# fhausmann/deepgrp

Hardware: AMD Instinct MI355X
Metric: Mbp/sec predicted (whole node) at window=200 stride=50, 5-class (higher is better)
Workload: dtype f16

## Files before the change

deepgrp_amd/csrc/gru_split2.hip:

```cpp
#include "gru_shared.h"
#include <mutex>
#include <type_traits>

typedef unsigned u32x4 __attribute__((ext_vector_type(4)));

namespace {

constexpr int NW = 4, UP = 128, KS = 4, HPAD = 16, HS = UP + HPAD;
constexpr int XT_PITCH = 4 * 128 * 4 + 32;

struct split2_weights {
    u32x4 hi[3][KS][2], lo[3][KS][2];
    u32x4 Bd_hi, Bd_lo;
};

#define LOAD2(a, pa, b, pb)                                                                                             \
    asm volatile("global_load_dwordx4 %0, %2, off\n\tglobal_load_dwordx4 %1, %3, off\n\ts_waitcnt vmcnt(0)"            \
                 : "=&a"(a), "=&a"(b) : "v"(pa), "v"(pb) : "memory")

#define MFMA_R(acc, Wf, b) asm volatile("v_mfma_f32_16x16x32_f16 %0, %1, %2, %0" : "+v"(acc) : "a"(Wf), "v"(b))
#define MFMA_D(acc, a, Wf) asm volatile("v_mfma_f32_16x16x32_f16 %0, %1, %2, %0" : "+v"(acc) : "v"(a), "a"(Wf))
#define MFMA_DZ(acc, a, Wf) asm volatile("v_mfma_f32_16x16x32_f16 %0, %1, %2, 0" : "=&v"(acc) : "v"(a), "a"(Wf))

struct tile_state {
    gru_params p;
    wg_ctx ctx;
    unsigned hcur, hnxt, lcur, lnxt;
    unsigned myseq;
    float h[16];
    f32x4 ar[4], ag[4], az[4], ax[4];
    f32x4 dpl;
    unsigned tabf, tabr;
    half8 f0h[2], f0l[2];
    int p_off;
    int64_t p_row0;
    bool pr_on;
};

template <int MODE, bool ONERCP>
__global__ void __launch_bounds__(256) __attribute__((amdgpu_waves_per_eu(1, 1))) gru_split2_kernel(const gru_params pin, int half_bytes)
{
    extern __shared__ __attribute__((aligned(16))) unsigned char smem[];
    const int tid = threadIdx.x;
    const int lane = tid & 63;
    const int wave = __builtin_amdgcn_readfirstlane(tid >> 6);
    const int T = pin.T, C = pin.C;

    split2_weights W;
    {
        const uint4 *p16 = pin.pack16 + (size_t)wave * 48 * 64 + lane;
#pragma unroll
        for (int g = 0; g < 3; ++g)
#pragma unroll
            for (int ks = 0; ks < KS; ++ks) {
                LOAD2(W.hi[g][ks][0], p16 + (size_t)(g * 8 + ks * 2) * 64, W.hi[g][ks][1], p16 + (size_t)(g * 8 + ks * 2 + 1) * 64);
                LOAD2(W.lo[g][ks][0], p16 + (size_t)(24 + g * 8 + ks * 2) * 64, W.lo[g][ks][1], p16 + (size_t)(24 + g * 8 + ks * 2 + 1) * 64);
            }
        const uint4 *mypack = pin.pack + (size_t)wave * pin.nfrag * 64 + lane;
        LOAD2(W.Bd_hi, mypack + (size_t)(3 * (2 * KS + 1) + 1) * 64, W.Bd_lo, mypack + (size_t)(3 * (2 * KS + 1) + 2) * 64);
    }
    for (int i = tid; i < 5 * 512; i += 256)
        *reinterpret_cast<float *>(smem + pin.xtab_off + (i / 512) * XT_PITCH + (i % 512) * 4) = pin.xtab[i];

    const int wi = lane & 15, q4 = lane >> 4;
    const int cls = lane & 15;
    const float fbias = cls < C ? pin.ffb[cls] : 0.0f;
    const int pwi = 4 * (lane >> 4) + wave;
    const unsigned frag_lane = (unsigned)(wi * HS + 8 * q4) * 2;
    const unsigned dense_lane = (unsigned)(wi * HS + 32 * wave + 8 * q4) * 2;
    const unsigned pub_lane = (unsigned)(wi * HS + 32 * wave + 4 * q4) * 2;
    const unsigned tab_lane = (unsigned)pin.xtab_off + (unsigned)(32 * wave + 4 * q4) * 4;

    tile_state S0, S1;
    auto setup = [&](tile_state &Z, int x) {
        unsigned char *base = smem + (size_t)x * half_bytes;
        _Float16 *lbuf = reinterpret_cast<_Float16 *>(base + pin.lo_tile_off);
        for (int i = tid; i < 32 * HS; i += 256) lbuf[i] = (_Float16)0.0f;
        Z.p = pin;
        const int64_t bid = wg_record_at<MODE>(pin, Z.p, 2 * (int64_t)blockIdx.x + x);
        Z.ctx = wg_setup<NW, MODE, HPAD>(Z.p, base, bid);
        Z.hcur = (unsigned)x * half_bytes;
        Z.hnxt = Z.hcur + 32 * HS * 2;
        Z.lcur = (unsigned)x * half_bytes + pin.lo_tile_off;
        Z.lnxt = Z.lcur + 32 * HS * 2;
        Z.myseq = (unsigned)(Z.ctx.seqs - smem) + wi * pin.Tp;
#pragma unroll
        for (int i = 0; i < 16; ++i) Z.h[i] = ONERCP ? -1.0f : 0.0f;
        Z.p_off = Z.ctx.rowoff[pwi];
        Z.p_row0 = Z.ctx.row0s[pwi];
        Z.pr_on = cls < C && pwi < Z.ctx.nvalid;
    };
    setup(S0, 0);
    setup(S1, 1);

    auto lds16 = [&](unsigned off) -> half8 { return *reinterpret_cast<const half8 *>(smem + off); };
    auto ldsf4 = [&](unsigned off) -> f32x4 { return *reinterpret_cast<const f32x4 *>(smem + off); };
    auto tab_rows = [&](tile_state &Z, uint32_t bf, uint32_t br) {
        bf = bf < 4 ? bf : 4;
        br = br < 4 ? 3 - br : 4;
        Z.tabf = tab_lane + bf * XT_PITCH;
        Z.tabr = tab_lane + br * XT_PITCH;
    };
    auto acc_init = [&](tile_state &Z, int g, int sub) {
        const f32x4 v = ldsf4(((sub & 1) ? Z.tabr : Z.tabf) + g * 512 + (sub >> 1) * 64);
        if (g == 0) Z.ar[sub] = v; else if (g == 1) Z.ag[sub] = v; else Z.az[sub] = v;
    };

    struct frag_ring { half8 h[2][2], l[2][2]; };
    struct dense_ops { half8 a0, a1, l0, l1; };
    struct fin_state { float d[NW], lg, m, e, s; };
    auto phase = [&](auto do_x, auto do_y, auto do_f, tile_state &X, tile_state &Y, int tx, int ty) __attribute__((always_inline)) {
        constexpr bool DO_X = decltype(do_x)::value, DO_Y = decltype(do_y)::value, DO_F = decltype(do_f)::value;
        frag_ring F;
        dense_ops D;
        fin_state fs;
        split_gate_tmp gt[16];
        float pbh[4][4];
        uint2 pbhv[4], pblv[4];
        uint32_t xp_bf = 4, xp_br = 4;
        const int td = ty - 1;
        const int tf = tx - 2;
        if constexpr (DO_X) { F.h[0][0] = X.f0h[0]; F.h[0][1] = X.f0h[1]; F.l[0][0] = X.f0l[0]; F.l[0][1] = X.f0l[1]; }
#define GAP __builtin_amdgcn_sched_barrier(0);
#define M_K(ks, n)                                                                                               \
    if constexpr (DO_X) {                                                                                        \
        constexpr int ps_ = (n) / 12, g_ = ((n) % 12) / 4, uh_ = ((n) % 4) / 2, rh_ = (n) % 2, sub_ = 2 * uh_ + rh_; \
        const half8 &b_ = ps_ == 1 ? F.l[(ks) & 1][rh_] : F.h[(ks) & 1][rh_];                                    \
        const u32x4 &w_ = ps_ == 2 ? W.lo[g_][ks][uh_] : W.hi[g_][ks][uh_];                                      \
        if constexpr (g_ == 0) MFMA_R(X.ar[sub_], w_, b_);                                                       \
        else if constexpr (g_ == 1) MFMA_R(X.ag[sub_], w_, b_);                                                  \
        else MFMA_R(X.az[sub_], w_, b_);                                                                         \
    }
#define M_D(i)                                                                                                   \
    if constexpr (DO_X) {                                                                                        \
        if constexpr ((i) == 0) MFMA_DZ(X.dpl, D.a0, W.Bd_hi);                                                   \
        else if constexpr ((i) == 1) MFMA_D(X.dpl, D.a1, W.Bd_hi);                                               \
        else if constexpr ((i) == 2) MFMA_D(X.dpl, D.a0, W.Bd_lo);                                               \
        else if constexpr ((i) == 3) MFMA_D(X.dpl, D.a1, W.Bd_lo);                                               \
        else if constexpr ((i) == 4) MFMA_D(X.dpl, D.l0, W.Bd_hi);                                               \
        else MFMA_D(X.dpl, D.l1, W.Bd_hi);                                                                       \
    }
#define PF(ks)                                                                                                   \
    if constexpr (DO_X) {                                                                                        \
        F.h[(ks) & 1][0] = lds16(X.hcur + frag_lane + 64 * (ks)); F.h[(ks) & 1][1] = lds16(X.hcur + frag_lane + 16 * HS * 2 + 64 * (ks)); \
        F.l[(ks) & 1][0] = lds16(X.lcur + frag_lane + 64 * (ks)); F.l[(ks) & 1][1] = lds16(X.lcur + frag_lane + 16 * HS * 2 + 64 * (ks)); \
    }
#define RDD                                                                                                      \
    if constexpr (DO_X) {                                                                                        \
        D.a0 = lds16(X.hcur + dense_lane); D.a1 = lds16(X.hcur + dense_lane + 16 * HS * 2);                      \
        D.l0 = lds16(X.lcur + dense_lane); D.l1 = lds16(X.lcur + dense_lane + 16 * HS * 2);                      \
        if (MODE == 2 && tx > 0 && (lane & 15) < X.ctx.nvalid)                                                   \
            split_avg_store(X.p, X.ctx.wg_w, tx - 1, UP, wave, D.a0, D.a1, D.l0, D.l1);                          \
    }
#define AXL(sub) \
    if constexpr (DO_Y) Y.ax[sub] = ldsf4((((sub) & 1) ? Y.tabr : Y.tabf) + 3 * 512 + ((sub) >> 1) * 64);
#define DS(i)                                                                                                    \
    if constexpr (DO_Y) Y.ctx.dpart[((size_t)(td & 1) * 4 * NW + wave) * 64 + lane + (i) * NW * 64] = Y.dpl[i];
#define G(e, op) \
    if constexpr (DO_Y) split_gate_op<ONERCP, op>(gt[e], Y.ar[(e) / 4][(e) % 4], Y.ag[(e) / 4][(e) % 4], Y.az[(e) / 4][(e) % 4], Y.ax[(e) / 4][(e) % 4], Y.h[e]);
#define PB(g, op)                                                                                                \
    if constexpr (DO_Y) {                                                                                        \
        if constexpr ((op) == 0) {                                                                               \
            pbh[g][0] = split_state_h<ONERCP>(Y.h[4 * (g)]); pbh[g][1] = split_state_h<ONERCP>(Y.h[4 * (g) + 1]); \
            pbh[g][2] = split_state_h<ONERCP>(Y.h[4 * (g) + 2]); pbh[g][3] = split_state_h<ONERCP>(Y.h[4 * (g) + 3]); \
        } else if constexpr ((op) == 1) {                                                                        \
            pbhv[g] = split_pack4(pbh[g]);                                                                       \
        } else if constexpr ((op) == 2) {                                                                        \
            split_residual4(pbh[g], pbhv[g]);                                                                    \
        } else if constexpr ((op) == 3) {                                                                        \
            pblv[g] = split_pack4(pbh[g]);                                                                       \
        } else {                                                                                                 \
            *reinterpret_cast<uint2 *>(smem + Y.hnxt + pub_lane + ((g) & 1) * 16 * HS * 2 + ((g) >> 1) * 32) = pbhv[g]; \
            *reinterpret_cast<uint2 *>(smem + Y.lnxt + pub_lane + ((g) & 1) * 16 * HS * 2 + ((g) >> 1) * 32) = pblv[g]; \
        }                                                                                                        \
    }
#define BAR                                                                                                      \
    if constexpr (DO_Y) {                                                                                        \
        asm volatile("s_waitcnt lgkmcnt(0)\n\ts_barrier" ::: "memory");                                          \
        unsigned sw_ = Y.hcur; Y.hcur = Y.hnxt; Y.hnxt = sw_;                                                    \
        sw_ = Y.lcur; Y.lcur = Y.lnxt; Y.lnxt = sw_;                                                             \
    }
#define RD0                                                                                                      \
    if constexpr (DO_Y) {                                                                                        \
        Y.f0h[0] = lds16(Y.hcur + frag_lane); Y.f0h[1] = lds16(Y.hcur + frag_lane + 16 * HS * 2);                \
        Y.f0l[0] = lds16(Y.lcur + frag_lane); Y.f0l[1] = lds16(Y.lcur + frag_lane + 16 * HS * 2);                \
    }
#define XP(op)                                                                                                   \
    if constexpr (DO_Y) {                                                                                        \
        if constexpr ((op) == 0) { xp_bf = smem[Y.myseq + ty + 1]; xp_br = smem[Y.myseq + T - 2 - ty]; }                       \
        else tab_rows(Y, xp_bf, xp_br);                                                                          \
    }
#define CI(g, sub) \
    if constexpr (DO_Y) acc_init(Y, g, sub);
#define FN(op)                                                                                                   \
    if constexpr (DO_F) {                                                                                        \
        if constexpr ((op) == 0) {                                                                               \
            const float *dp_ = X.ctx.dpart + ((size_t)(tf & 1) * 4 + wave) * NW * 64 + lane;                     \
            fs.d[0] = dp_[0]; fs.d[1] = dp_[64]; fs.d[2] = dp_[128]; fs.d[3] = dp_[192];                         \
        } else if constexpr ((op) == 1) {                                                                        \
            const float sum_ = ((fs.d[0] + fs.d[1]) + fs.d[2]) + fs.d[3];                                        \
            fs.lg = cls < C ? sum_ + fbias : -INFINITY;                                                          \
        } else if constexpr ((op) == 2) { if (MODE != 2) fs.m = row_max_ror<8>(fs.lg); }                         \
        else if constexpr ((op) == 3) { if (MODE != 2) fs.m = row_max_ror<4>(fs.m); }                            \
        else if constexpr ((op) == 4) { if (MODE != 2) fs.m = row_max_ror<2>(fs.m); }                            \
        else if constexpr ((op) == 5) { if (MODE != 2) fs.m = row_max_ror<1>(fs.m); }                            \
        else if constexpr ((op) == 6) { if (MODE != 2) fs.e = __builtin_amdgcn_exp2f(1.4426950408889634f * (fs.lg - fs.m)); } \
        else if constexpr ((op) == 7) { if (MODE != 2) fs.s = fs.e + row_ror<8>(fs.e); }                         \
        else if constexpr ((op) == 8) { if (MODE != 2) fs.s += row_ror<4>(fs.s); }                               \
        else if constexpr ((op) == 9) { if (MODE != 2) fs.s += row_ror<2>(fs.s); }                               \
        else if constexpr ((op) == 10) { if (MODE != 2) fs.s += row_ror<1>(fs.s); }                              \
        else if constexpr ((op) == 11) { if (MODE != 2) fs.e *= __builtin_amdgcn_rcpf(fs.s); }                   \
        else { if (X.pr_on && tf >= 0) emit_value<MODE>(X.p, X.ctx, X.p_off, X.p_row0, tf, cls, MODE == 2 ? fs.lg : fs.e); } \
    }
#include "gru_split2_phase.inc"
#undef GAP
#undef M_K
#undef M_D
#undef PF
#undef RDD
#undef AXL
#undef DS
#undef G
#undef PB
#undef BAR
#undef RD0
#undef XP
#undef CI
#undef FN
    };
    const std::true_type yes;
    const std::false_type no;

    auto first_step = [&](tile_state &Z) {
        tab_rows(Z, smem[Z.myseq], smem[Z.myseq + T - 1]);
#pragma unroll
        for (int g = 0; g < 3; ++g)
#pragma unroll
            for (int sub = 0; sub < 4; ++sub) acc_init(Z, g, sub);
        Z.f0h[0] = lds16(Z.hcur + frag_lane); Z.f0h[1] = lds16(Z.hcur + frag_lane + 16 * HS * 2);
        Z.f0l[0] = lds16(Z.lcur + frag_lane); Z.f0l[1] = lds16(Z.lcur + frag_lane + 16 * HS * 2);
    };
    first_step(S0);
    first_step(S1);
    phase(yes, no, no, S0, S1, 0, 0);
#define EDGE_PAD do { asm volatile("s_nop 15\n\ts_nop 7"); __builtin_amdgcn_sched_barrier(0); } while (0)
    EDGE_PAD;
    for (int t = 0; t + 1 < T; ++t) {
        phase(yes, yes, yes, S1, S0, t, t);
        phase(yes, yes, yes, S0, S1, t + 1, t);
        EDGE_PAD;
    }
    phase(yes, yes, yes, S1, S0, T - 1, T - 1);
    phase(no, yes, yes, S0, S1, T, T - 1);

    auto drain = [&](tile_state &Z, bool prev_open) {
        const half8 a0 = lds16(Z.hcur + dense_lane), a1 = lds16(Z.hcur + dense_lane + 16 * HS * 2);
        const half8 l0 = lds16(Z.lcur + dense_lane), l1 = lds16(Z.lcur + dense_lane + 16 * HS * 2);
        if (MODE == 2 && (lane & 15) < Z.ctx.nvalid) split_avg_store(Z.p, Z.ctx.wg_w, T - 1, UP, wave, a0, a1, l0, l1);
        f32x4 d;
        MFMA_DZ(d, a0, W.Bd_hi); MFMA_D(d, a1, W.Bd_hi); MFMA_D(d, a0, W.Bd_lo); MFMA_D(d, a1, W.Bd_lo); MFMA_D(d, l0, W.Bd_hi); MFMA_D(d, l1, W.Bd_hi);
        asm volatile("s_nop 15\n\ts_nop 7" : "+v"(d));
        float *dw = Z.ctx.dpart + ((size_t)((T - 1) & 1) * 4 * NW + wave) * 64 + lane;
#pragma unroll
        for (int reg = 0; reg < 4; ++reg) dw[reg * NW * 64] = d[reg];
        __syncthreads();
        if (prev_open && T > 1) finish_register<NW, MODE>(Z.p, Z.ctx, T - 2, wave, fbias, Z.p_off, Z.p_row0);
        finish_register<NW, MODE>(Z.p, Z.ctx, T - 1, wave, fbias, Z.p_off, Z.p_row0);
        if (MODE == 0 && pin.ospan > 0) flush_image<NW>(Z.p, Z.ctx);
    };
    drain(S0, false);
    drain(S1, true);
}

template <int MODE, bool ONERCP>
int launch_split2(const gru_params &p, int64_t groups, int half_bytes, hipStream_t stream)
{
    static std::once_flag configured;
    static hipError_t cfg_err = hipSuccess;
    std::call_once(configured, [] { cfg_err = hipFuncSetAttribute((const void *)gru_split2_kernel<MODE, ONERCP>, hipFuncAttributeMaxDynamicSharedMemorySize, 160 * 1024); });
    DGRP_HIP(cfg_err);
    hipLaunchKernelGGL((gru_split2_kernel<MODE, ONERCP>), dim3((unsigned)((groups + 1) / 2)), dim3(256), (size_t)2 * half_bytes + 5 * XT_PITCH, stream, p, half_bytes);
    DGRP_LAUNCH_CHECK();
    return DGRP_OK;
}

}

int dgrp_split2_launch(const gru_params &p, int64_t groups, int half_bytes, bool onercp, hipStream_t stream)
{
    if (onercp)
        return p.mode == 0 ? launch_split2<0, true>(p, groups, half_bytes, stream)
             : p.mode == 1 ? launch_split2<1, true>(p, groups, half_bytes, stream) : launch_split2<2, true>(p, groups, half_bytes, stream);
    return p.mode == 0 ? launch_split2<0, false>(p, groups, half_bytes, stream)
         : p.mode == 1 ? launch_split2<1, false>(p, groups, half_bytes, stream) : launch_split2<2, false>(p, groups, half_bytes, stream);
}
```

Baseline: 550.2.

## Overlap GRU kernel prologue loads with LDS setup and batch weight loads

Restructures the kernel prologue. The global loads of the x-table and the sequence bytes are issued early into registers and committed to LDS after the weight loads. The weight fragments now load in batches of sixteen dwordx4 per asm block instead of pairs with a wait after each pair, and the wg_setup call is inlined into separate place, fill, row and commit stages with 16-byte zero fills. This aims to hide prologue memory latency before the recurrent loop, at the cost of more register pressure during the prologue and more complex sequence-staging code. It also adds optional timestamp instrumentation, compiled only under a define.

```diff
diff --git a/deepgrp_amd/csrc/gru_split2.hip b/deepgrp_amd/csrc/gru_split2.hip
--- a/deepgrp_amd/csrc/gru_split2.hip
+++ b/deepgrp_amd/csrc/gru_split2.hip
@@ -37,6 +37,25 @@
     bool pr_on;
 };
 
+#ifdef DGRP_SPLIT2_STAMPS
+#define SPLIT2_STAMP(k)                                                                                          \
+    do {                                                                                                         \
+        __builtin_amdgcn_sched_barrier(0);                                                                       \
+        if (MODE == 0 && pin.avg) {                                                                              \
+            unsigned long long c_, r_;                                                                           \
+            asm volatile("s_memtime %0\n\ts_memrealtime %1\n\ts_waitcnt lgkmcnt(0)" : "=s"(c_), "=s"(r_) :: "memory"); \
+            if (threadIdx.x == 0) {                                                                              \
+                unsigned long long *b_ = reinterpret_cast<unsigned long long *>(pin.avg) + (size_t)blockIdx.x * 16; \
+                b_[2 * (k)] = c_; b_[2 * (k) + 1] = r_;                                                          \
+                if ((k) == 0) { b_[10] = __builtin_amdgcn_s_getreg(4 | (31 << 11)); b_[11] = __builtin_amdgcn_s_getreg(20 | (31 << 11)); } \
+            }                                                                                                    \
+        }                                                                                                        \
+        __builtin_amdgcn_sched_barrier(0);                                                                       \
+    } while (0)
+#else
+#define SPLIT2_STAMP(k) do { } while (0)
+#endif
+
 template <int MODE, bool ONERCP>
 __global__ void __launch_bounds__(256) __attribute__((amdgpu_waves_per_eu(1, 1))) gru_split2_kernel(const gru_params pin, int half_bytes)
 {
@@ -46,25 +65,9 @@
     const int wave = __builtin_amdgcn_readfirstlane(tid >> 6);
     const int T = pin.T, C = pin.C;
 
-    split2_weights W;
-    {
-        const uint4 *p16 = pin.pack16 + (size_t)wave * 48 * 64 + lane;
-#pragma unroll
-        for (int g = 0; g < 3; ++g)
-#pragma unroll
-            for (int ks = 0; ks < KS; ++ks) {
-                LOAD2(W.hi[g][ks][0], p16 + (size_t)(g * 8 + ks * 2) * 64, W.hi[g][ks][1], p16 + (size_t)(g * 8 + ks * 2 + 1) * 64);
-                LOAD2(W.lo[g][ks][0], p16 + (size_t)(24 + g * 8 + ks * 2) * 64, W.lo[g][ks][1], p16 + (size_t)(24 + g * 8 + ks * 2 + 1) * 64);
-            }
-        const uint4 *mypack = pin.pack + (size_t)wave * pin.nfrag * 64 + lane;
-        LOAD2(W.Bd_hi, mypack + (size_t)(3 * (2 * KS + 1) + 1) * 64, W.Bd_lo, mypack + (size_t)(3 * (2 * KS + 1) + 2) * 64);
-    }
-    for (int i = tid; i < 5 * 512; i += 256)
-        *reinterpret_cast<float *>(smem + pin.xtab_off + (i / 512) * XT_PITCH + (i % 512) * 4) = pin.xtab[i];
-
+    SPLIT2_STAMP(0);
     const int wi = lane & 15, q4 = lane >> 4;
     const int cls = lane & 15;
-    const float fbias = cls < C ? pin.ffb[cls] : 0.0f;
     const int pwi = 4 * (lane >> 4) + wave;
     const unsigned frag_lane = (unsigned)(wi * HS + 8 * q4) * 2;
     const unsigned dense_lane = (unsigned)(wi * HS + 32 * wave + 8 * q4) * 2;
@@ -72,26 +75,173 @@
     const unsigned tab_lane = (unsigned)pin.xtab_off + (unsigned)(32 * wave + 4 * q4) * 4;
 
     tile_state S0, S1;
-    auto setup = [&](tile_state &Z, int x) {
+    auto place = [&](tile_state &Z, int x) {
         unsigned char *base = smem + (size_t)x * half_bytes;
-        _Float16 *lbuf = reinterpret_cast<_Float16 *>(base + pin.lo_tile_off);
-        for (int i = tid; i < 32 * HS; i += 256) lbuf[i] = (_Float16)0.0f;
         Z.p = pin;
         const int64_t bid = wg_record_at<MODE>(pin, Z.p, 2 * (int64_t)blockIdx.x + x);
-        Z.ctx = wg_setup<NW, MODE, HPAD>(Z.p, base, bid);
+        wg_ctx &c = Z.ctx;
+        c.hbuf = reinterpret_cast<_Float16 *>(base);
+        c.dpart = reinterpret_cast<float *>(base + gru_lds_hbuf(UP, HPAD));
+        c.seqs = base + gru_lds_hbuf(UP, HPAD) + gru_lds_dpart(NW);
+        c.row0s = reinterpret_cast<int64_t *>(c.seqs + gru_lds_seq(pin.Tp));
+        c.rowoff = reinterpret_cast<int *>(c.row0s + DGRP_WG_WINDOWS);
+        c.obuf = reinterpret_cast<unsigned *>(c.rowoff + DGRP_WG_WINDOWS);
+        c.wg_w = Z.p.w0 + bid * DGRP_WG_WINDOWS;
+        c.nvalid = (int)min((int64_t)DGRP_WG_WINDOWS, Z.p.w0 + Z.p.nw - c.wg_w);
+        c.lo = 0;
+        if (MODE == 0) {
+            const int64_t a = dgrp_place_row(Z.p.place, c.wg_w, Z.p.s), b = dgrp_place_row(Z.p.place, c.wg_w + c.nvalid - 1, Z.p.s);
+            c.lo = a < b ? a : b;
+        }
         Z.hcur = (unsigned)x * half_bytes;
         Z.hnxt = Z.hcur + 32 * HS * 2;
         Z.lcur = (unsigned)x * half_bytes + pin.lo_tile_off;
         Z.lnxt = Z.lcur + 32 * HS * 2;
+    };
+    place(S0, 0);
+    place(S1, 1);
+
+    constexpr int SEQ_R = 2;
+    const bool span_form = pin.s <= (int64_t)T && 15 * pin.s + 2 * (int64_t)T + 16 <= (int64_t)gru_lds_seq(pin.Tp);
+    struct seq_regs { uint32_t dw[SEQ_R]; uint8_t by; };
+    auto seq_geom = [&](const tile_state &Z, const uint8_t *&g4, int &al, int &len) {
+        const int nv = Z.ctx.nvalid > 0 ? Z.ctx.nvalid : 0;
+        const uint8_t *g = Z.p.idx + Z.ctx.wg_w * Z.p.s;
+        al = (int)(reinterpret_cast<uintptr_t>(g) & 3);
+        g4 = g - al;
+        len = nv > 0 ? (nv - 1) * (int)Z.p.s + T : 0;
+    };
+    auto seq_issue = [&](const tile_state &Z, seq_regs &Q) {
+        const uint8_t *g4; int al, len;
+        seq_geom(Z, g4, al, len);
+#pragma unroll
+        for (int r = 0; r < SEQ_R; ++r) {
+            const int k = tid + 256 * r;
+            Q.dw[r] = 0;
+            if (4 * k >= al && 4 * k + 4 <= al + len) Q.dw[r] = reinterpret_cast<const uint32_t *>(g4)[k];
+        }
+        const int kl = (al + len - 1) >> 2, k = tid < 4 ? 0 : kl, j = 4 * k + (tid & 3) - al;
+        Q.by = 0;
+        if (tid < 8 && (tid < 4 || kl > 0) && j >= 0 && j < len && !(4 * k >= al && 4 * k + 4 <= al + len)) Q.by = g4[al + j];
+    };
+    auto seq_commit = [&](tile_state &Z, const seq_regs &Q) {
+        const uint8_t *g4; int al, len;
+        seq_geom(Z, g4, al, len);
+        unsigned char *dst = Z.ctx.seqs + 4;
+#pragma unroll
+        for (int r = 0; r < SEQ_R; ++r) {
+            const int k = tid + 256 * r;
+            if (4 * k >= al && 4 * k + 4 <= al + len) reinterpret_cast<uint32_t *>(dst)[k] = Q.dw[r];
+        }
+        const int kl = (al + len - 1) >> 2, k = tid < 4 ? 0 : kl, j = 4 * k + (tid & 3) - al;
+        if (tid < 8 && (tid < 4 || kl > 0) && j >= 0 && j < len && !(4 * k >= al && 4 * k + 4 <= al + len)) dst[al + j] = Q.by;
+        for (int k0 = 256 * SEQ_R; 4 * k0 < al + len; k0 += 4 * 256) {
+            uint32_t v[4];
+#pragma unroll
+            for (int r = 0; r < 4; ++r) {
+                const int kk = k0 + tid + 256 * r;
+                v[r] = 4 * kk + 4 <= al + len ? reinterpret_cast<const uint32_t *>(g4)[kk] : 0u;
+            }
+#pragma unroll
+            for (int r = 0; r < 4; ++r) {
+                const int kk = k0 + tid + 256 * r;
+                if (4 * kk + 4 <= al + len) reinterpret_cast<uint32_t *>(dst)[kk] = v[r];
+            }
+        }
+        const int fours = (al + len + 3) & ~3;
+        for (int i = tid; 4 * i < T; i += 256) reinterpret_cast<uint32_t *>(dst + fours)[i] = 0x04040404u;
+        Z.myseq = (unsigned)(dst - smem) + (wi < Z.ctx.nvalid ? al + wi * (int)Z.p.s : fours);
+    };
+    auto seq_rows = [&](tile_state &Z) {
+        const int w = tid >> 4;
+        const bool on = w < Z.ctx.nvalid;
+        const uint8_t *g = Z.p.idx + (Z.ctx.wg_w + w) * Z.p.s;
+        for (int t0 = tid & 15; t0 < T; t0 += 8 * 16) {
+            uint8_t v[8];
+#pragma unroll
+            for (int r = 0; r < 8; ++r) v[r] = on && t0 + 16 * r < T ? g[t0 + 16 * r] : (uint8_t)4;
+#pragma unroll
+            for (int r = 0; r < 8; ++r)
+                if (t0 + 16 * r < T) Z.ctx.seqs[w * pin.Tp + t0 + 16 * r] = v[r];
+        }
         Z.myseq = (unsigned)(Z.ctx.seqs - smem) + wi * pin.Tp;
+    };
+
+    const f32x4 *xsrc = reinterpret_cast<const f32x4 *>(pin.xtab) + tid;
+    const f32x4 xt0 = xsrc[0], xt1 = xsrc[256];
+    f32x4 xt2 = { 0.0f, 0.0f, 0.0f, 0.0f };
+    if (tid < 5 * 128 - 512) xt2 = xsrc[512];
+    seq_regs Q0, Q1;
+    if (span_form) { seq_issue(S0, Q0); seq_issue(S1, Q1); }
+    const float fbias = cls < C ? pin.ffb[cls] : 0.0f;
+    auto zero16 = [&](unsigned char *at, int bytes) {
+        for (int i = tid; i < bytes / 16; i += 256) reinterpret_cast<uint4 *>(at)[i] = uint4{ 0u, 0u, 0u, 0u };
+        if (tid < (bytes & 15) / 4) reinterpret_cast<unsigned *>(at + (bytes & ~15))[tid] = 0u;
+    };
+    auto fills = [&](tile_state &Z) {
+        zero16(smem + Z.hcur, 32 * HS * 2);
+        zero16(smem + Z.lcur, 32 * HS * 2);
+        if (MODE == 0) zero16(reinterpret_cast<unsigned char *>(Z.ctx.obuf), pin.ospan * C * 4);
+    };
+    fills(S0);
+    fills(S1);
+
+    split2_weights W;
+    {
+        const uint4 *p16 = pin.pack16 + (size_t)wave * 48 * 64 + lane;
+#define WF(f) ((f) < 24 ? W.hi[((f) % 24) / 8][((f) % 8) / 2][(f) % 2] : W.lo[((f) % 24) / 8][((f) % 8) / 2][(f) % 2])
+#define GLD(o, a, off) "global_load_dwordx4 %" #o ", %" #a ", off offset:" #off "\n\t"
+#define GLD8(o0, o1, o2, o3, o4, o5, o6, o7, a) \
+    GLD(o0, a, -4096) GLD(o1, a, -3072) GLD(o2, a, -2048) GLD(o3, a, -1024) GLD(o4, a, 0) GLD(o5, a, 1024) GLD(o6, a, 2048) GLD(o7, a, 3072)
+#define LOAD16(f)                                                                                                          \
+    asm volatile(GLD8(0, 1, 2, 3, 4, 5, 6, 7, 16) GLD8(8, 9, 10, 11, 12, 13, 14, 15, 17) "s_waitcnt vmcnt(0)"            \
+                 : "=&a"(WF((f) + 0)), "=&a"(WF((f) + 1)), "=&a"(WF((f) + 2)), "=&a"(WF((f) + 3)), "=&a"(WF((f) + 4)), "=&a"(WF((f) + 5)),     \
+                   "=&a"(WF((f) + 6)), "=&a"(WF((f) + 7)), "=&a"(WF((f) + 8)), "=&a"(WF((f) + 9)), "=&a"(WF((f) + 10)), "=&a"(WF((f) + 11)),  \
+                   "=&a"(WF((f) + 12)), "=&a"(WF((f) + 13)), "=&a"(WF((f) + 14)), "=&a"(WF((f) + 15))                     \
+                 : "v"(p16 + (size_t)((f) + 4) * 64), "v"(p16 + (size_t)((f) + 12) * 64) : "memory")
+        LOAD16(0);
+        LOAD16(16);
+        LOAD16(32);
+#undef LOAD16
+#undef GLD8
+#undef GLD
+#undef WF
+        const uint4 *mypack = pin.pack + (size_t)wave * pin.nfrag * 64 + lane;
+        LOAD2(W.Bd_hi, mypack + (size_t)(3 * (2 * KS + 1) + 1) * 64, W.Bd_lo, mypack + (size_t)(3 * (2 * KS + 1) + 2) * 64);
+    }
+    SPLIT2_STAMP(1);
+
+    auto xrow = [&](int i) { return reinterpret_cast<f32x4 *>(smem + pin.xtab_off + (i >> 7) * XT_PITCH + (i & 127) * 16); };
+    *xrow(tid) = xt0;
+    *xrow(tid + 256) = xt1;
+    if (tid < 5 * 128 - 512) *xrow(tid + 512) = xt2;
+    if (span_form) { seq_commit(S0, Q0); seq_commit(S1, Q1); }
+    else { seq_rows(S0); seq_rows(S1); }
+    auto rows = [&](tile_state &Z) {
+        const wg_ctx &c = Z.ctx;
+        if (tid < DGRP_WG_WINDOWS) {
+            int64_t r0 = -1;
+            int off = -1;
+            if (tid < c.nvalid) {
+                r0 = MODE == 0 ? dgrp_place_row(Z.p.place, c.wg_w + tid, Z.p.s) : (c.wg_w + tid - Z.p.w0 + Z.p.avgw) * (int64_t)T;
+                if (MODE == 0 && r0 >= c.lo && r0 - c.lo + T <= pin.ospan) off = (int)(r0 - c.lo);
+            }
+            c.row0s[tid] = r0;
+            c.rowoff[tid] = off;
+        }
+    };
+    rows(S0);
+    rows(S1);
+    __syncthreads();
+    auto start = [&](tile_state &Z) {
 #pragma unroll
         for (int i = 0; i < 16; ++i) Z.h[i] = ONERCP ? -1.0f : 0.0f;
         Z.p_off = Z.ctx.rowoff[pwi];
         Z.p_row0 = Z.ctx.row0s[pwi];
         Z.pr_on = cls < C && pwi < Z.ctx.nvalid;
     };
-    setup(S0, 0);
-    setup(S1, 1);
+    start(S0);
+    start(S1);
 
     auto lds16 = [&](unsigned off) -> half8 { return *reinterpret_cast<const half8 *>(smem + off); };
     auto ldsf4 = [&](unsigned off) -> f32x4 { return *reinterpret_cast<const f32x4 *>(smem + off); };
@@ -242,6 +392,7 @@
     };
     first_step(S0);
     first_step(S1);
+    SPLIT2_STAMP(2);
     phase(yes, no, no, S0, S1, 0, 0);
 #define EDGE_PAD do { asm volatile("s_nop 15\n\ts_nop 7"); __builtin_amdgcn_sched_barrier(0); } while (0)
     EDGE_PAD;
@@ -252,6 +403,7 @@
     }
     phase(yes, yes, yes, S1, S0, T - 1, T - 1);
     phase(no, yes, yes, S0, S1, T, T - 1);
+    SPLIT2_STAMP(3);
 
     auto drain = [&](tile_state &Z, bool prev_open) {
         const half8 a0 = lds16(Z.hcur + dense_lane), a1 = lds16(Z.hcur + dense_lane + 16 * HS * 2);
@@ -270,7 +422,13 @@
     };
     drain(S0, false);
     drain(S1, true);
+    SPLIT2_STAMP(4);
 }
+
+#ifdef DGRP_SPLIT2_STAMPS
+void *stamp_buf = nullptr;
+long long stamp_wgs = 0;
+#endif
 
 template <int MODE, bool ONERCP>
 int launch_split2(const gru_params &p, int64_t groups, int half_bytes, hipStream_t stream)
@@ -279,7 +437,13 @@
     static hipError_t cfg_err = hipSuccess;
     std::call_once(configured, [] { cfg_err = hipFuncSetAttribute((const void *)gru_split2_kernel<MODE, ONERCP>, hipFuncAttributeMaxDynamicSharedMemorySize, 160 * 1024); });
     DGRP_HIP(cfg_err);
+#ifdef DGRP_SPLIT2_STAMPS
+    gru_params q = p;
+    if (MODE == 0) q.avg = (groups + 1) / 2 <= stamp_wgs ? stamp_buf : nullptr;
+    hipLaunchKernelGGL((gru_split2_kernel<MODE, ONERCP>), dim3((unsigned)((groups + 1) / 2)), dim3(256), (size_t)2 * half_bytes + 5 * XT_PITCH, stream, q, half_bytes);
+#else
     hipLaunchKernelGGL((gru_split2_kernel<MODE, ONERCP>), dim3((unsigned)((groups + 1) / 2)), dim3(256), (size_t)2 * half_bytes + 5 * XT_PITCH, stream, p, half_bytes);
+#endif
     DGRP_LAUNCH_CHECK();
     return DGRP_OK;
 }
@@ -294,3 +458,11 @@
     return p.mode == 0 ? launch_split2<0, false>(p, groups, half_bytes, stream)
          : p.mode == 1 ? launch_split2<1, false>(p, groups, half_bytes, stream) : launch_split2<2, false>(p, groups, half_bytes, stream);
 }
+
+#ifdef DGRP_SPLIT2_STAMPS
+extern "C" __attribute__((visibility("default"))) int dgrp_split2_stamp_buffer(void *dev, long long wgs)
+{
+    stamp_buf = dev; stamp_wgs = dev ? wgs : 0;
+    return DGRP_OK;
+}
+#endif
```

Result: no change. 553.5 (median of 6 runs) (+0.6%).
